# smups/inflatox

Hardware: AMD Instinct MI355X
Metric: grid-points/sec on complete_analysis sweep; achieved HBM GB/s vs peak (higher is better)
Workload: dtype f64

## Files before the change

### inflatox_amd/_native.py

```python

from __future__ import annotations

import ctypes as C
import os
import subprocess

import numpy as np

_PKG = os.path.dirname(os.path.abspath(__file__))
_REPO = os.path.dirname(_PKG)
LIB_PATH = os.path.join(_PKG, "libinflx_hip.so")

OK, ERR_IO, ERR_SYMBOL, ERR_VERSION, ERR_SHAPE, ERR_DEVICE, ERR_ARG, ERR_BASIS, ERR_GSL = range(9)
SF_EDOM, SF_EDECLINED = 1, 2
SF_QUIET, SF_FAIL = 0, 1

OP_COMPLETE, OP_CONSISTENCY, OP_RAPIDTURN, OP_EPSILON_V, OP_RAW = range(5)
OP_HESSE = 6
OP_QDIF = 5
OP_GROUP = {OP_COMPLETE: "core", OP_CONSISTENCY: "consistency", OP_RAPIDTURN: "rapidturn", OP_EPSILON_V: "epsilon_v", OP_RAW: "raw", OP_QDIF: "qdif", OP_HESSE: "hesse"}
OP_WIDTH = {OP_COMPLETE: 6, OP_CONSISTENCY: 1, OP_RAPIDTURN: 1, OP_EPSILON_V: 1, OP_RAW: 5, OP_HESSE: 4}
LAYOUT_AOS, LAYOUT_SOA = 0, 1
SWEEP_DEFAULT, SWEEP_FORCE_TILE = 0, 1
TIME_BACK_TO_BACK, TIME_DOMINANT_ONLY, TIME_IN_PIPELINE, TIME_SINGLE_CALL = range(4)
# ... 40 lines not shown
        C.c_int,
        [C.c_void_p, C.c_int, _DP, _SIZE, _SIZE, C.c_void_p, _SIZE, _DP, _SIZE, _SIZE, _SIZE, _SIZE, C.c_int, C.c_void_p, C.c_int, C.c_int, C.c_uint, C.POINTER(C.c_float)],
    ),
    "inflx_sweep_plan_ex": (C.c_int, [C.c_void_p, C.c_int, _SIZE, _SIZE, _SIZE, C.c_int, C.c_uint, C.POINTER(C.c_uint32)]),
    "inflx_host_threads": (C.c_int, [C.c_uint, C.POINTER(C.c_uint)]),
    "inflx_sweep_device_stats": (
        C.c_int,
        [C.c_void_p, _DP, _SIZE, _SIZE, C.c_void_p, _SIZE, _DP, _SIZE, _SIZE, _SIZE, _SIZE, C.c_void_p, C.c_void_p],
    ),
    "inflx_synchronize": (C.c_int, [C.c_void_p]),
    "inflx_sf_status": (C.c_int, [C.c_void_p, C.POINTER(C.c_uint), C.c_int]),
    "inflx_sf_policy": (C.c_int, [C.c_void_p, C.c_int]),
    "inflx_uses_gsl": (C.c_int, [C.c_void_p]),
    "inflx_sweep_plan": (C.c_int, [C.c_void_p, C.c_int, _SIZE, _SIZE, _SIZE, C.c_int, C.POINTER(C.c_uint32)]),
    "inflx_basis_on_points": (C.c_int, [C.c_void_p, _DP, _SIZE, _DP, _SIZE, _DP]),
    "inflx_ops_on_values": (C.c_int, [C.c_void_p, _DP, _SIZE, _DP, C.c_int]),
    "inflx_validate_basis_at_random": (C.c_int, [C.c_void_p, C.c_uint64]),
    "inflx_validate_basis_on_domain": (C.c_int, [C.c_void_p, C.POINTER(C.c_uint32), _SIZE, _DP, _SIZE, _DP, C.c_double]),
    "inflx_shard_plan": (C.c_int, [_SIZE, _SIZE, C.c_int, C.c_int, C.POINTER(_SIZE)]),
    "inflx_open_multi": (C.c_int, [C.c_char_p, C.POINTER(C.c_int), C.c_int, C.POINTER(C.c_void_p)]),
    "inflx_close_multi": (None, [C.c_void_p]),
    "inflx_multi_device_count": (C.c_int, [C.c_void_p]),
    "inflx_multi_handle": (C.c_void_p, [C.c_void_p, C.c_int]),
    "inflx_sweep_host_multi": (C.c_int, [C.c_void_p, C.c_int, _DP, _SIZE, _SIZE, _DP, _DP, _SIZE, _SIZE, C.c_int, C.c_int, _SIZE]),
    "inflx_complete_analysis_multi": (C.c_int, [C.c_void_p, _DP, _SIZE, _DP, _DP, _SIZE, _SIZE, C.c_int, _SIZE]),
    "inflx_sweep_stats_multi": (C.c_int, [C.c_void_p, _DP, _SIZE, _SIZE, _DP, _SIZE, _SIZE, _SIZE, C.c_void_p]),
    "inflx_sweep_device_multi": (C.c_int, [C.c_void_p, C.c_int, _DP, _SIZE, _SIZE, C.POINTER(C.c_void_p), C.POINTER(_SIZE), _DP, _SIZE, _SIZE, C.c_int, C.POINTER(C.c_void_p)]),
    "inflx_sweep_allgather_multi": (C.c_int, [C.c_void_p, C.c_int, _DP, _SIZE, _SIZE, C.POINTER(C.c_void_p), _SIZE, _DP, _SIZE, _SIZE]),
    "inflx_sweep_allgather_multi_ex": (C.c_int, [C.c_void_p, C.c_int, _DP, _SIZE, _SIZE, C.POINTER(C.c_void_p), _SIZE, _DP, _SIZE, _SIZE, C.c_int]),
    "inflx_solve_eom": (
        C.c_int,
        [C.c_void_p, _DP, _SIZE, _SIZE, _DP, _SIZE, _SIZE, _SIZE, C.c_int, C.c_double, C.c_double, C.c_uint, _DP, _DP, _DP, C.POINTER(C.c_int8), C.POINTER(C.c_int64)],
    ),
    "inflx_solve_eom_to_efolds": (
        C.c_int,
        [C.c_void_p, _DP, _SIZE, _SIZE, _DP, _SIZE, _DP, _SIZE, C.c_int, C.c_double, C.c_double, C.c_uint, _DP, _DP, _DP, _DP, C.POINTER(C.c_int8)],
    ),
    "inflx_solve_eom_sampled": (
        C.c_int,
        [C.c_void_p, _DP, _SIZE, _SIZE, _DP, _SIZE, _DP, _SIZE, _SIZE, C.c_int, C.c_double, C.c_double, C.c_uint, _DP, _DP, C.POINTER(C.c_int8), C.POINTER(C.c_uint32)],
    ),
}


class Summary(C.Structure):

    _fields_ = [("min", C.c_double * 6), ("max", C.c_double * 6), ("count", C.c_uint64 * 6)]

_lib = None


def build_library(force: bool = False) -> str:
    src = os.path.join(_PKG, "csrc", "inflx_hip.cpp")
    deps = [src, os.path.join(_PKG, "csrc", "inflx_kernel_abi.h"), os.path.join(_PKG, "csrc", "inflx_background_abi.h"), os.path.join(_REPO, "include", "inflx_hip.h")]
    stale = force or not os.path.exists(LIB_PATH) or any(os.path.getmtime(d) > os.path.getmtime(LIB_PATH) for d in deps)
    if stale:
        from .compiler import hipcc_path

        cmd = [
            hipcc_path(),
            "-O2",
            "-fPIC",
            "-shared",
            "-std=c++17",
            "-Wall",
            "-Wextra",
            f"-I{os.path.join(_REPO, 'include')}",
            f"-I{os.path.join(_PKG, 'csrc')}",
            src,
            "-o",
            LIB_PATH + ".tmp",
        ]
        subprocess.run(cmd, check=True)
        os.replace(LIB_PATH + ".tmp", LIB_PATH)
    return LIB_PATH


def _preload_hip_runtime():
    import importlib.util

    try:
        spec = importlib.util.find_spec("torch")
    except (ImportError, ValueError):
        spec = None
    if spec is not None and spec.origin:
        cand = os.path.join(os.path.dirname(spec.origin), "lib", "libamdhip64.so")
        if os.path.exists(cand):
            C.CDLL(cand, mode=C.RTLD_GLOBAL)


def load_library():
    global _lib
    if _lib is None:
        if not os.path.exists(LIB_PATH):
            raise ImportError(
                f"{LIB_PATH} is missing: build it with `python -c 'import __graft_entry__ as g; g.build()'` "
                "(the sweep has no CPU fallback)"
            )
        _preload_hip_runtime()
        lib = C.CDLL(LIB_PATH)
        for name, (res, args) in SIGNATURES.items():
            fn = getattr(lib, name)
            fn.restype = res
            fn.argtypes = args
        _lib = lib
    return _lib


class InflatoxShapeError(Exception):
    """Counterpart of LibInflxRsErr::Shape, which PyO3 raises as a plain Exception (err.rs:71)."""


class InflatoxBasisError(Exception):
    """Counterpart of LibInflxRsErr::BasisNorm / BasisOth (err.rs:36-37), plain Exceptions in PyO3 too."""


class InflatoxSpecialFunctionError(ArithmeticError):
    """A special function of the model was called outside its domain somewhere in the call (``INFLX_ERR_GSL``).  The reference's
    GSL error handler prints the reason and panics at that point (src/err.rs:86-103): the call does not return there either.  Here
    the result was complete when the error was raised -- NaN at the offending points -- and ``sf_errors="nan"`` returns it."""


def _raise(rc: int):
    msg = load_library().inflx_last_error().decode("utf-8", "replace")
    if rc == ERR_GSL:
        raise InflatoxSpecialFunctionError(msg)
    if rc == ERR_IO:
        raise IOError(msg)
# ... 469 lines not shown
```

### inflatox_amd/csrc/inflx_hip.cpp

```cpp
#include "inflx_hip.h"

#include <dlfcn.h>
#include <hip/hip_runtime.h>

#include <algorithm>
#include <atomic>
#include <cerrno>
#include <chrono>
#include <cmath>
#include <cstdarg>
#include <cstdio>
#include <cstdlib>
#include <condition_variable>
#include <cstring>
#include <mutex>
#include <future>
#include <random>
#include <string>
#include <thread>
#include <vector>

#include <sched.h>
#include <sys/mman.h>
#if defined(__x86_64__)
#include <emmintrin.h>
#endif
#include <unistd.h>

#include "inflx_background_abi.h"
#include "inflx_kernel_abi.h"

namespace {

thread_local std::string g_last_error;

int fail(int code, const char* fmt, ...) {
  char buf[1024];
  va_list ap;
  va_start(ap, fmt);
  vsnprintf(buf, sizeof buf, fmt, ap);
  va_end(ap);
  g_last_error = buf;
  return code;
}

#define HIP_TRY(expr)                                                                              \
  do {                                                                                             \
    hipError_t e_ = (expr);                                                                        \
    if (e_ != hipSuccess) return fail(INFLX_ERR_DEVICE, "%s failed: %s", #expr, hipGetErrorString(e_)); \
  } while (0)

constexpr uint16_t kAbiMajor = 5, kAbiMinor = 0;
const char* const kOpNames[INFLX_OP_COUNT] = {"complete", "consistency", "rapidturn", "epsilon_v", "raw", "qdif", "hesse"};
constexpr int kOpWidth[INFLX_OP_COUNT] = {6, 1, 1, 1, 5, 1, 4};
constexpr size_t kOpBytes[INFLX_OP_COUNT] = {48, 8, 8, 8, 40, 1, 32};

size_t chunk_bytes_limit() {
  static const size_t v = [] {
    const char* e = getenv("INFLX_CHUNK_MB");
    const long mb = e ? atol(e) : 0;
    return (size_t)(mb > 0 ? mb : 32) << 20;
  }();
  return v;
}
size_t whole_result_limit() {
  static const size_t v = [] {
    const char* e = getenv("INFLX_WHOLE_RESULT_MB");
    const long mb = e ? atol(e) : -1;
    return (size_t)(mb >= 0 ? mb : 65536) << 20;
  }();
  return v;
}
unsigned quota_from(const std::string& quota_file, const std::string& period_file) {
  FILE* fh = fopen(quota_file.c_str(), "r");
  if (!fh) return 0;
  char a[64] = {0}, b[64] = {0};
  const int got = fscanf(fh, "%63s %63s", a, b);
  fclose(fh);
  if (got < 1 || strcmp(a, "max") == 0) return 0;
  double quota = atof(a), period = got >= 2 ? atof(b) : 0.0;
  if (!period_file.empty()) {
    FILE* ph = fopen(period_file.c_str(), "r");
    if (!ph) return 0;
// ... 151 lines not shown
      }
    }
    if (!spawned) work(a, b);
  }
  for (auto& th : pool) th.join();
}

struct TableRing {
  double* buf[2] = {nullptr, nullptr};
  size_t cap[2] = {0, 0};
  hipEvent_t ready[2] = {nullptr, nullptr};
  hipEvent_t free[2] = {nullptr, nullptr};
  bool used[2] = {false, false};
  unsigned turn = 0;

  bool create() {
    for (int b = 0; b < 2; ++b)
      if (hipEventCreateWithFlags(&ready[b], hipEventDisableTiming | hipEventDisableSystemFence) != hipSuccess ||
          hipEventCreateWithFlags(&free[b], hipEventDisableTiming | hipEventDisableSystemFence) != hipSuccess)
        return false;
    return true;
  }
  void destroy() {
    for (int b = 0; b < 2; ++b) {
      if (ready[b]) (void)hipEventDestroy(ready[b]);
      if (free[b]) (void)hipEventDestroy(free[b]);
      if (buf[b]) (void)hipFree(buf[b]);
    }
  }
  bool idle() const {
    for (int b = 0; b < 2; ++b)
      if (used[b] && hipEventQuery(free[b]) != hipSuccess) return false;
    return true;
  }
  int grow(int b, size_t doubles) {
    if (buf[b]) HIP_TRY(hipFree(buf[b]));
    buf[b] = nullptr;
    cap[b] = 0;
    HIP_TRY(hipMalloc(reinterpret_cast<void**>(&buf[b]), doubles * sizeof(double)));
    cap[b] = doubles;
    return INFLX_OK;
  }
};
}

#define INFLX_SERIALISE(m) \
  std::unique_lock<std::recursive_mutex> inflx_call_lock_; \
  if (m) inflx_call_lock_ = std::unique_lock<std::recursive_mutex>((m)->mu)

struct inflx_model {
  std::recursive_mutex mu;
  int device = 0;
  hipModule_t module = nullptr;
  hipStream_t stream = nullptr;
  hipStream_t copy_stream = nullptr;
  hipFunction_t tile[INFLX_OP_COUNT] = {};
  hipFunction_t rows[INFLX_OP_COUNT] = {};
  hipFunction_t traj[INFLX_OP_COUNT] = {};
  hipFunction_t basis_points = nullptr;
  hipFunction_t ops_on_values = nullptr;
  hipFunction_t rowvals[INFLX_OP_COUNT] = {};
  hipFunction_t rowstream6 = nullptr;
  hipFunction_t rowstream_planes = nullptr;
  hipFunction_t colvals[INFLX_OP_COUNT] = {};
  hipFunction_t colstream = nullptr;
  hipFunction_t colvals_stats = nullptr;
  hipFunction_t stage_tables = nullptr;
  TableRing stage_ring;
  hipFunction_t tile_stats = nullptr, tile_stats_nostore = nullptr, rowvals_stats = nullptr;
  double* d_stats = nullptr;
  TableRing row_ring;
  hipStream_t side = nullptr;
  std::vector<std::pair<hipEvent_t, hipEvent_t>>* probe = nullptr;
  size_t probe_used = 0;
  bool probe_overflow = false;
  InflxKernelInfo info = {};
  uint32_t groups = 0;
  std::vector<hipModule_t> attached;
  std::string tag;
  std::vector<hipDeviceptr_t> sf_words;
  int sf_policy = INFLX_SF_QUIET;
  hipEvent_t sf_done = nullptr;
  bool sf_pending = false;
  char use_gsl = 0;
  uint16_t version[3] = {};
  uint32_t dim = 0, n_par = 0;
  std::string name, path;
  struct ParamSlot {
    double* host = nullptr;
    double* dev = nullptr;
    size_t cap = 0, count = 0;
    hipStream_t stream = nullptr;
    hipEvent_t last_use = nullptr;
    hipStream_t last_reader = nullptr;
    bool in_flight = false;
  };
  static constexpr int kParamSlots = 4;
  ParamSlot pslot[kParamSlots];
  int pcur = 0;
  void* d_chunk[2] = {nullptr, nullptr};
  size_t d_chunk_cap[2] = {0, 0};
  void* d_whole = nullptr;
  size_t d_whole_cap = 0;
  hipEvent_t chunk_done[2] = {nullptr, nullptr};
  hipEvent_t copy_done[2] = {nullptr, nullptr};
  hipEvent_t t0 = nullptr, t1 = nullptr;
// ... 71 lines not shown

void note_sf_word(inflx_model* m, hipModule_t module) {
  if (!m->use_gsl) return;
  hipDeviceptr_t dptr = nullptr;
  size_t size = 0;
  if (hipModuleGetGlobal(&dptr, &size, module, "INFLX_SF_STATUS") == hipSuccess && size == sizeof(unsigned))
    m->sf_words.push_back(dptr);
  else
    (void)hipGetLastError();
}

int sf_collect(inflx_model* m, bool clear, unsigned* bits) {
  *bits = 0;
  if (m->sf_words.empty()) return INFLX_OK;
  HIP_TRY(hipSetDevice(m->device));
  HIP_TRY(hipStreamSynchronize(m->side));
  HIP_TRY(hipStreamSynchronize(m->stream));
  if (m->sf_pending) {
    HIP_TRY(hipEventSynchronize(m->sf_done));
    m->sf_pending = false;
  }
  for (hipDeviceptr_t w : m->sf_words) {
    unsigned v = 0;
    HIP_TRY(hipMemcpy(&v, w, sizeof v, hipMemcpyDeviceToHost));
    *bits |= v;
    if (v && clear) {
      const unsigned zero = 0;
      HIP_TRY(hipMemcpy(w, &zero, sizeof zero, hipMemcpyHostToDevice));
    }
  }
  return INFLX_OK;
}

int sf_error(const inflx_model* m, unsigned bits) {
  const bool dom = (bits & INFLX_SF_EDOM) != 0;
  return fail(INFLX_ERR_GSL, "a GSL exception ocurred (ERRCODE %s): model \"%s\" called a special function %s at one or more points of this call. "
              "Those points hold NaN and the result is complete otherwise; the reference's GSL error handler panics here instead of returning. "
              "inflx_sf_policy(handle, INFLX_SF_QUIET) / GeneralisedAL(..., sf_errors=\"nan\") returns the result with its NaNs.",
              dom ? "0X1" : "0X11", m->name.c_str(),
              dom ? "outside its domain (input domain error)" : "where this implementation could not deliver 1e-13 and declined (loss of accuracy)");
}

int sf_verdict(inflx_model* m) {
  if (m->sf_words.empty() || m->sf_policy != INFLX_SF_FAIL) return INFLX_OK;
  unsigned bits = 0;
  const int rc = sf_collect(m, true, &bits);
  if (rc) return rc;
  return bits ? sf_error(m, bits) : INFLX_OK;
}

const char* const kGroupNames[9] = {"core", "stats", "values", "consistency", "rapidturn", "epsilon_v", "raw", "qdif", "hesse"};
uint32_t group_of_op(int op) { return INFLX_GROUP_OF_OP(op); }

int resolve_group_kernels(inflx_model* m, hipModule_t module, uint32_t mask, const char* path) {
  auto get = [&](hipFunction_t* slot, const std::string& name) -> int {
    if (hipModuleGetFunction(slot, module, name.c_str()) != hipSuccess) {
      *slot = nullptr;
      return fail(INFLX_ERR_SYMBOL, "artefact %s lacks kernel %s", path, name.c_str());
    }
    return INFLX_OK;
  };
  int rc;
  for (int op = 0; op < INFLX_OP_COUNT; ++op) {
    if (!(mask & group_of_op(op))) continue;
    const std::string nm = kOpNames[op];
    if ((rc = get(&m->tile[op], "inflx_sweep_tile_" + nm)) || (rc = get(&m->rows[op], "inflx_sweep_rows_" + nm)) || (rc = get(&m->traj[op], "inflx_sweep_traj_" + nm)) ||
        (rc = get(&m->rowvals[op], "inflx_sweep_rowvals_" + nm)) || (rc = get(&m->colvals[op], "inflx_sweep_colvals_" + nm)))
      return rc;
  }
  if (mask & INFLX_GROUP_CORE) {
    if ((rc = get(&m->rowstream6, "inflx_sweep_rowstream6")) || (rc = get(&m->rowstream_planes, "inflx_sweep_rowstream_planes")) || (rc = get(&m->colstream, "inflx_sweep_colstream")) ||
        (rc = get(&m->stage_tables, "inflx_stage_tables")) || (rc = get(&m->basis_points, "inflx_basis_points")))
      return rc;
  }
  if (mask & INFLX_GROUP_STATS) {
    if ((rc = get(&m->tile_stats, "inflx_sweep_tile_complete_stats")) || (rc = get(&m->tile_stats_nostore, "inflx_sweep_tile_complete_stats_nostore")) ||
        (rc = get(&m->rowvals_stats, "inflx_sweep_rowvals_complete_stats")) || (rc = get(&m->colvals_stats, "inflx_sweep_colvals_complete_stats")))
      return rc;
  }
  if (mask & INFLX_GROUP_VALUES) {
    if ((rc = get(&m->ops_on_values, "inflx_ops_on_values"))) return rc;
  }
  return INFLX_OK;
}

template <typename T>
int read_global_of(hipModule_t module, const char* path, const char* sym, T* dst, size_t bytes, bool exact) {
  hipDeviceptr_t dptr = nullptr;
  size_t size = 0;
  if (hipModuleGetGlobal(&dptr, &size, module, sym) != hipSuccess) return fail(INFLX_ERR_SYMBOL, "artefact %s lacks symbol %s", path, sym);
  if (exact ? size != bytes : size > bytes) return fail(INFLX_ERR_SYMBOL, "symbol %s in %s has %zu bytes, expected %s%zu", sym, path, size, exact ? "" : "<= ", bytes);
  HIP_TRY(hipMemcpy(dst, dptr, size, hipMemcpyDeviceToHost));
  return INFLX_OK;
}

int attach_object(inflx_model* m, const char* path) {
  hipModule_t module = nullptr;
  hipError_t e = hipModuleLoad(&module, path);
  if (e != hipSuccess) return fail(INFLX_ERR_IO, "could not load %s as a gfx950 code object: %s", path, hipGetErrorString(e));
  auto bail = [&](int code) {
    const std::string first = g_last_error;
    (void)hipModuleUnload(module);
    g_last_error = first;
    return code;
  };
  uint16_t version[3] = {};
  InflxKernelInfo info = {};
  uint32_t groups = 0;
  char tag[128] = {0};
  int rc;
  if ((rc = read_global_of(module, path, "VERSION", version, sizeof version, true)) || (rc = read_global_of(module, path, "INFLX_KERNEL_INFO", &info, sizeof info, true)) ||
      (rc = read_global_of(module, path, "INFLX_GROUPS", &groups, sizeof groups, true)) || (rc = read_global_of(module, path, "MODEL_TAG", tag, sizeof tag - 1, false)))
    return bail(rc);
  if (version[0] != m->version[0] || version[1] != m->version[1] || memcmp(&info, &m->info, sizeof info) != 0 || m->tag != tag)
    return bail(fail(INFLX_ERR_VERSION, "%s does not belong to artefact %s: built from another model, with other options or for another kernel ABI (tag \"%s\", expected \"%s\")",
                     path, m->path.c_str(), tag, m->tag.c_str()));
  const uint32_t fresh = groups & ~m->groups;
  if ((rc = resolve_group_kernels(m, module, fresh, path))) return bail(rc);
  m->attached.push_back(module);
  m->groups |= fresh;
  note_sf_word(m, module);
  return INFLX_OK;
}

int need_groups(inflx_model* m, uint32_t mask) {
// ... 61 lines not shown
    pl.cpr = (units_row + info.row_chunk_units - 1) / info.row_chunk_units;
    pl.replicas = 32;
    while (pl.replicas > 1 && pl.replicas > pl.cpr) pl.replicas /= 2;
    const size_t line_bytes = row_count * pl.replicas * 64;
    pl.batch = std::max<size_t>(1, std::min<size_t>(P, (size_t(64) << 20) / std::max<size_t>(line_bytes, 1)));
    pl.batch = std::min<size_t>(pl.batch, 65535 / (aos6 ? 1 : K));
    pl.one_stream = alone && P <= pl.batch;
  } else if (col_only && (planes ? N1 : K * N1) % 2 == 0) {
    pl.path = INFLX_PATH_COL_STREAM;
    pl.batch = std::max<size_t>(1, std::min<size_t>(P, (size_t(64) << 20) / std::max<size_t>(K * N1 * 8, 1)));
    pl.batch = std::min<size_t>(pl.batch, 65535 / (planes ? K : 1));
    pl.one_stream = alone && P <= pl.batch;
  } else if (row_only) {
    pl.path = INFLX_PATH_ROWS;
  } else {
    pl.path = INFLX_PATH_TILE;
    const size_t nu = std::max<size_t>(info.n_uniform, 1), nc = std::max<size_t>(info.n_col, 1);
    const size_t nr = (std::max<size_t>(info.n_row, 1) + 1) & ~size_t(1);
    pl.rows_per_launch = size_t(65535) * info.tile_rows;
    const size_t per_p = nu + std::min(pl.rows_per_launch, row_count) * nr + nc * N1;
    pl.batch = std::max<size_t>(1, std::min<size_t>(P, (size_t(1) << 27) / std::max<size_t>(per_p, 1)));
    pl.one_stream = alone && P <= pl.batch && row_count <= pl.rows_per_launch;
  }
  return pl;
}

bool handle_idle(inflx_model* m) {
  const bool idle = m->row_ring.idle() && m->stage_ring.idle();
  (void)hipGetLastError();
  return idle;
}

hipError_t probe_begin(inflx_model* m, hipStream_t s) {
  if (!m->probe) return hipSuccess;
  if (m->probe_used >= m->probe->size()) {
    m->probe_overflow = true;
    return hipSuccess;
  }
  return hipEventRecord((*m->probe)[m->probe_used].first, s);
}
hipError_t probe_end(inflx_model* m, hipStream_t s) {
  if (!m->probe || m->probe_used >= m->probe->size()) return hipSuccess;
  return hipEventRecord((*m->probe)[m->probe_used++].second, s);
}


struct BroadcastPath {
  hipFunction_t eval;
  unsigned eval_gx, eval_block;
  hipFunction_t store;
  size_t cpr;
  size_t z_per_p;
  size_t table_doubles;
};

int launch_broadcast(inflx_model* m, const SweepPlan& plan, const BroadcastPath& path, int op, InflxSweepArgs a, const double* d_params, size_t P,
                     double* d_out, hipStream_t s, bool stores_only) {
  void* params[] = {&a};
  TableRing& ring = m->row_ring;
  const hipStream_t ev = plan.upload_stream(m, s);
  const size_t batch = plan.batch, row_count = a.row_count;
  if (path.cpr > 0x7fffffffULL) return fail(INFLX_ERR_SHAPE, "grid rows too long for one launch");
  if (stores_only && batch < P)
    return fail(INFLX_ERR_ARG, "dominant_only timing needs the parameter rows to fit one table batch (%zu rows here, got %zu)", batch, P);
  const bool store = d_out != nullptr;
  for (size_t p0 = 0; p0 < P; p0 += batch) {
    const size_t pb = std::min(batch, P - p0);
    const int b = (int)((ring.turn + (stores_only ? 1 : 0)) & 1);
    if (store && pb * path.table_doubles > ring.cap[b]) {
      HIP_TRY(hipDeviceSynchronize());
      const int rc = ring.grow(b, pb * path.table_doubles);
      if (rc) return rc;
    }
    a.params = d_params + p0 * m->n_par;
    a.out = store ? d_out + p0 * row_count * a.N1 * kOpWidth[op] : nullptr;
    a.P = (uint32_t)pb;
    a.row_table = store ? ring.buf[b] : nullptr;
    if (!stores_only) {
      if (ring.used[b]) HIP_TRY(hipStreamWaitEvent(ev, ring.free[b], 0));
      HIP_TRY(hipModuleLaunchKernel(path.eval, path.eval_gx, (unsigned)pb, 1, path.eval_block, 1, 1, 0, ev, params, nullptr));
      if (ev != s) HIP_TRY(hipEventRecord(ring.ready[b], ev));
      ring.turn++;
    }
    if (store) {
      if (ev != s) HIP_TRY(hipStreamWaitEvent(s, ring.ready[b], 0));
      for (size_t r0 = 0; r0 < row_count; r0 += 65535) {
        a.stream_row0 = (uint32_t)r0;
        const size_t nr = std::min<size_t>(65535, row_count - r0);
        HIP_TRY(probe_begin(m, s));
        HIP_TRY(hipModuleLaunchKernel(path.store, (unsigned)path.cpr, (unsigned)nr, (unsigned)(pb * path.z_per_p), m->info.tile_cols, 1, 1, 0, s, params, nullptr));
        HIP_TRY(probe_end(m, s));
      }
      HIP_TRY(hipEventRecord(ring.free[b], s));
      ring.used[b] = true;
    }
  }
  return INFLX_OK;
}

int launch_rows_fallback(inflx_model* m, int op, InflxSweepArgs a, size_t P, size_t N1, size_t row_count, hipStream_t s) {
  void* params[] = {&a};
  const size_t rpb = m->info.rows_per_block;
  const size_t groups = (row_count + rpb - 1) / rpb;
  size_t chunks = 1;
  const size_t want = 4096;
  if (groups * P < want) {
    const size_t units = N1 / 64;
    chunks = std::min<size_t>(std::max<size_t>(units, 1), (want + groups * P - 1) / (groups * P));
  }
  if (groups * chunks > 0x7fffffffULL) return fail(INFLX_ERR_SHAPE, "grid too large for one launch");
  a.col_chunks = (uint32_t)chunks;
  HIP_TRY(hipModuleLaunchKernel(m->rows[op], (unsigned)(groups * chunks), (unsigned)P, 1, m->info.tile_cols, 1, 1, 0, s, params,
                                nullptr));
  return INFLX_OK;
}

constexpr size_t kLaunchWorkgroups = 1024;

size_t tile_height(size_t full, size_t segments) {
  return std::min(full, std::max<size_t>({size_t(1), std::min(full / 2, segments / kLaunchWorkgroups), segments / (4 * kLaunchWorkgroups)}));
}

int launch_tiles(inflx_model* m, const SweepPlan& plan, int op, InflxSweepArgs a, const double* d_params, size_t P, double* d_out, size_t N1,
                 size_t row_count, hipStream_t s, double* d_stats) {
  void* params[] = {&a};
  TableRing& ring = m->stage_ring;
  const size_t gx = (N1 + m->info.tile_cols - 1) / m->info.tile_cols;
  if (gx > 0x7fffffffULL) return fail(INFLX_ERR_SHAPE, "grid rows too long for one launch (%zu column tiles)", gx);
  if (row_count > 0xffffffffULL) return fail(INFLX_ERR_SHAPE, "at most 2^32 grid rows per call (got %zu)", row_count);
  hipFunction_t f = d_stats ? (d_out ? m->tile_stats : m->tile_stats_nostore) : m->tile[op];
  const size_t nu = std::max<size_t>(m->info.n_uniform, 1), nc = std::max<size_t>(m->info.n_col, 1);
  const size_t nr = (std::max<size_t>(m->info.n_row, 1) + 1) & ~size_t(1);
  const size_t rows_per_launch = plan.rows_per_launch, pbatch = plan.batch;
  const hipStream_t tables = plan.upload_stream(m, s);
  for (size_t p0 = 0; p0 < P; p0 += pbatch) {
    const size_t pb = std::min(pbatch, P - p0);
    a.params = d_params + p0 * m->n_par;
    a.out = d_out ? reinterpret_cast<double*>(reinterpret_cast<char*>(d_out) + p0 * row_count * N1 * kOpBytes[op]) : nullptr;
    a.P = (uint32_t)pb;
    for (size_t r0 = 0; r0 < row_count; r0 += rows_per_launch) {
      const size_t slab = std::min(rows_per_launch, row_count - r0);
      const size_t need = pb * (nu + slab * nr + nc * N1);
      const int b = (int)(ring.turn & 1);
// ... 10 lines not shown
      HIP_TRY(hipModuleLaunchKernel(m->stage_tables, (unsigned)tx, (unsigned)pb, 1, m->info.tile_cols, 1, 1, 0, tables, params, nullptr));
      ring.turn++;
      if (tables != s) {
        HIP_TRY(hipEventRecord(ring.ready[b], tables));
        HIP_TRY(hipStreamWaitEvent(s, ring.ready[b], 0));
      }
      const size_t th = tile_height(m->info.tile_rows, gx * slab * pb);
      a.tile_rows = (uint32_t)th;
      const size_t gy = (slab + th - 1) / th;
      HIP_TRY(probe_begin(m, s));
      HIP_TRY(hipModuleLaunchKernel(f, (unsigned)gx, (unsigned)gy, (unsigned)pb, m->info.tile_cols, 1, 1, 0, s, params, nullptr));
      HIP_TRY(probe_end(m, s));
      HIP_TRY(hipEventRecord(ring.free[b], s));
      ring.used[b] = true;
    }
  }
  return INFLX_OK;
}

int launch_grid(inflx_model* m, const SweepPlan& plan, int op, const double* d_params, size_t P, double* d_out, const double* ss, size_t N0,
                size_t N1, size_t row_begin, size_t row_count, int layout, hipStream_t s, bool stores_only = false, double accuracy = 0.0,
                double* d_stats = nullptr) {
  if (row_count == 0 || N1 == 0) return INFLX_OK;
  if (P > 65535) {
    for (size_t p0 = 0; p0 < P; p0 += 65535) {
      const size_t pb = std::min<size_t>(65535, P - p0);
      double* sub = d_out ? reinterpret_cast<double*>(reinterpret_cast<char*>(d_out) + p0 * row_count * N1 * kOpBytes[op]) : nullptr;
      const int rc = launch_grid(m, plan, op, d_params + p0 * m->n_par, pb, sub, ss, N0, N1, row_begin, row_count, layout, s, stores_only, accuracy, d_stats);
      if (rc) return rc;
    }
    return INFLX_OK;
  }
  InflxSweepArgs a;
  memset(&a, 0, sizeof a);
  a.out = d_out;
  a.params = d_params;
  a.x0a = ss[0];
  a.dx0 = (ss[1] - ss[0]) / (double)N0;
  a.x1a = ss[2];
  a.dx1 = (ss[3] - ss[2]) / (double)N1;
  a.N1 = N1;
  a.row_begin = row_begin;
  a.row_count = row_count;
  a.P = (uint32_t)P;
  a.layout = (uint32_t)layout;
  a.col_chunks = 1;
  a.accuracy = accuracy;
  a.stats = d_stats;
  const size_t K = kOpWidth[op];
  switch (plan.path) {
    case INFLX_PATH_ROW_STREAM: {
      const bool aos6 = K == 6 && layout == INFLX_AOS;
      a.table_replicas = (uint32_t)plan.replicas;
      a.stream_planes = (uint32_t)K;
      const BroadcastPath path = {d_stats ? m->rowvals_stats : m->rowvals[op], (unsigned)((row_count + 63) / 64), 64,
                                  aos6 ? m->rowstream6 : m->rowstream_planes, plan.cpr, aos6 ? 1 : K, row_count * plan.replicas * 8};
      return launch_broadcast(m, plan, path, op, a, d_params, P, d_out, s, stores_only);
    }
    case INFLX_PATH_COL_STREAM: {
      const bool planes = layout == INFLX_SOA || K == 1;
      a.stream_units = (planes ? N1 : K * N1) / 2;
      const size_t tc = m->info.tile_cols;
      const BroadcastPath path = {d_stats ? m->colvals_stats : m->colvals[op], (unsigned)((N1 + tc - 1) / tc), (unsigned)tc,
                                  m->colstream, (a.stream_units + tc - 1) / tc, planes ? K : 1, K * N1};
      return launch_broadcast(m, plan, path, op, a, d_params, P, d_out, s, stores_only);
    }
    case INFLX_PATH_ROWS:
      return launch_rows_fallback(m, op, a, P, N1, row_count, s);
    default:
      return launch_tiles(m, plan, op, a, d_params, P, d_out, N1, row_count, s, d_stats);
  }
}

int ensure_chunk(inflx_model* m, int which, size_t bytes) {
  if (bytes <= m->d_chunk_cap[which]) return INFLX_OK;
  if (m->d_chunk[which]) HIP_TRY(hipFree(m->d_chunk[which]));
  m->d_chunk[which] = nullptr;
  m->d_chunk_cap[which] = 0;
  HIP_TRY(hipMalloc(&m->d_chunk[which], bytes));
  m->d_chunk_cap[which] = bytes;
  return INFLX_OK;
}

void say(const char* fmt, ...) {
  va_list ap;
  va_start(ap, fmt);
  fputs("[Inflatox Info] ", stderr);
  vfprintf(stderr, fmt, ap);
  fputc('\n', stderr);
  fflush(stderr);
  va_end(ap);
}

void warn(const char* fmt, ...) {
  va_list ap;
  va_start(ap, fmt);
  fputs("[Inflatox Warning] ", stderr);
  vfprintf(stderr, fmt, ap);
  fputc('\n', stderr);
  fflush(stderr);
  va_end(ap);
}

std::string num_text(double v, int digits = -1) {
  if (std::isnan(v)) return "NaN";
  if (std::isinf(v)) return v > 0 ? "inf" : "-inf";
  char buf[64];
  if (digits >= 0) snprintf(buf, sizeof buf, "%.*f", digits, v); else snprintf(buf, sizeof buf, "%.17g", v);
  return buf;
}

std::string list_text(const double* v, size_t n) {
  std::string s = "[";
  for (size_t k = 0; k < n; ++k) s += (k ? ", " : "") + num_text(v[k], 3);
  return s + "]";
}

// ... 69 lines not shown
  if (device < 0 || device >= ndev) return fail(INFLX_ERR_ARG, "device %d out of range (have %d)", device, ndev);
  HIP_TRY(hipSetDevice(device));

  inflx_model* m = new inflx_model();
  m->device = device;
  m->path = artefact_path;
  auto bail = [&](int code) {
    inflx_close(m);
    return code;
  };
  hipError_t e = hipModuleLoad(&m->module, artefact_path);
  if (e != hipSuccess) {
    m->module = nullptr;
    fail(INFLX_ERR_IO, "could not load %s as a gfx950 code object: %s", artefact_path, hipGetErrorString(e));
    return bail(INFLX_ERR_IO);
  }
  int rc;
  if ((rc = read_global(m, "VERSION", m->version, sizeof m->version, true))) return bail(rc);
  if (m->version[0] != kAbiMajor || m->version[1] != kAbiMinor) {
    fail(INFLX_ERR_VERSION, "artefact %s was built for inflatox ABI v%u.%u.%u, this library implements v%u.%u", artefact_path,
         m->version[0], m->version[1], m->version[2], kAbiMajor, kAbiMinor);
    return bail(INFLX_ERR_VERSION);
  }
  if ((rc = read_global(m, "DIM", &m->dim, sizeof m->dim, true))) return bail(rc);
  if ((rc = read_global(m, "N_PARAMETERS", &m->n_par, sizeof m->n_par, true))) return bail(rc);
  char name[512] = {0};
  if ((rc = read_global(m, "MODEL_NAME", name, sizeof name - 1, false))) return bail(rc);
  m->name = name;
  if ((rc = read_global(m, "INFLX_KERNEL_INFO", &m->info, sizeof m->info, true))) return bail(rc);
  if (m->info.kernel_abi != INFLX_KERNEL_ABI) {
    fail(INFLX_ERR_VERSION, "artefact %s uses kernel ABI %u, this library expects %u", artefact_path, m->info.kernel_abi,
         INFLX_KERNEL_ABI);
    return bail(INFLX_ERR_VERSION);
  }
  if ((rc = read_global(m, "USE_GSL", &m->use_gsl, sizeof m->use_gsl, true))) return bail(rc);
  note_sf_word(m, m->module);
  m->sf_policy = m->use_gsl ? INFLX_SF_FAIL : INFLX_SF_QUIET;
  char tag[128] = {0};
  if ((rc = read_global(m, "INFLX_GROUPS", &m->groups, sizeof m->groups, true))) return bail(rc);
  if ((rc = read_global(m, "MODEL_TAG", tag, sizeof tag - 1, false))) return bail(rc);
  m->tag = tag;
  m->groups &= INFLX_GROUP_ALL;
  if (!(m->groups & INFLX_GROUP_CORE)) {
    fail(INFLX_ERR_SYMBOL, "artefact %s is not a model's core object (it carries kernel groups 0x%x only): open the core object and attach this one (inflx_attach)", artefact_path, m->groups);
    m->groups = 0;
    return bail(INFLX_ERR_SYMBOL);
  }
  {
    const uint32_t present = m->groups;
    m->groups = 0;
    if ((rc = resolve_group_kernels(m, m->module, present, artefact_path))) return bail(rc);
    m->groups = present;
  }
  if (hipStreamCreateWithFlags(&m->stream, hipStreamNonBlocking) != hipSuccess ||
      hipStreamCreateWithFlags(&m->side, hipStreamNonBlocking) != hipSuccess ||
      hipStreamCreateWithFlags(&m->copy_stream, hipStreamNonBlocking) != hipSuccess) {
    fail(INFLX_ERR_DEVICE, "could not create HIP streams");
    return bail(INFLX_ERR_DEVICE);
  }
  for (int k = 0; k < 2; ++k) {
    if (hipEventCreateWithFlags(&m->chunk_done[k], hipEventDisableTiming) != hipSuccess ||
        hipEventCreateWithFlags(&m->copy_done[k], hipEventDisableTiming) != hipSuccess) {
      fail(INFLX_ERR_DEVICE, "could not create HIP events");
      return bail(INFLX_ERR_DEVICE);
    }
  }
  for (TableRing* ring : {&m->row_ring, &m->stage_ring}) {
    if (!ring->create()) {
      fail(INFLX_ERR_DEVICE, "could not create HIP events");
      return bail(INFLX_ERR_DEVICE);
    }
  }
  if (hipEventCreate(&m->t0) != hipSuccess || hipEventCreate(&m->t1) != hipSuccess) {
    fail(INFLX_ERR_DEVICE, "could not create HIP timing events");
    return bail(INFLX_ERR_DEVICE);
  }
  *out = m;
  return INFLX_OK;
}

void inflx_close(inflx_model* m) {
  if (!m) return;
  { std::lock_guard<std::recursive_mutex> last_call_has_returned(m->mu); }
  (void)hipSetDevice(m->device);
  if (m->stream) (void)hipStreamSynchronize(m->stream);
  if (m->side) (void)hipStreamSynchronize(m->side);
  if (m->copy_stream) (void)hipStreamSynchronize(m->copy_stream);
  for (int k = 0; k < 2; ++k) {
    if (m->d_chunk[k]) (void)hipFree(m->d_chunk[k]);
    if (m->chunk_done[k]) (void)hipEventDestroy(m->chunk_done[k]);
    if (m->copy_done[k]) (void)hipEventDestroy(m->copy_done[k]);
  }
  for (TableRing* ring : {&m->row_ring, &m->stage_ring}) ring->destroy();
  if (m->t0) (void)hipEventDestroy(m->t0);
  if (m->t1) (void)hipEventDestroy(m->t1);
  if (m->sf_done) (void)hipEventDestroy(m->sf_done);
  for (auto& slot : m->pslot) {
    if (slot.dev) (void)hipFree(slot.dev);
    if (slot.host) (void)hipHostFree(slot.host);
    if (slot.last_use) (void)hipEventDestroy(slot.last_use);
  }
  if (m->d_stats) (void)hipFree(m->d_stats);
  if (m->d_whole) (void)hipFree(m->d_whole);
  if (m->stream) (void)hipStreamDestroy(m->stream);
  if (m->side) (void)hipStreamDestroy(m->side);
  if (m->copy_stream) (void)hipStreamDestroy(m->copy_stream);
  for (hipModule_t extra : m->attached) (void)hipModuleUnload(extra);
  if (m->bg_module) (void)hipModuleUnload(m->bg_module);
  if (m->module) (void)hipModuleUnload(m->module);
  delete m;
}

int inflx_attach(inflx_model* m, const char* path) {
  if (!m || !path) return fail(INFLX_ERR_ARG, "model handle / path is NULL");
  INFLX_SERIALISE(m);
  FILE* fh = fopen(path, "rb");
  if (!fh) return fail(INFLX_ERR_IO, "could not open code object %s: %s", path, strerror(errno));
  fclose(fh);
  HIP_TRY(hipSetDevice(m->device));
  return attach_object(m, path);
}

uint32_t inflx_groups(const inflx_model* m) { return m ? m->groups : 0; }

uint32_t inflx_n_fields(const inflx_model* m) { return m ? m->dim : 0; }
uint32_t inflx_n_parameters(const inflx_model* m) { return m ? m->n_par : 0; }
const char* inflx_model_name(const inflx_model* m) { return m ? m->name.c_str() : ""; }
int inflx_device_of(const inflx_model* m) { return m ? m->device : -1; }

int inflx_host_threads(unsigned devices_at_work, unsigned out[3]) {
  if (!out) return fail(INFLX_ERR_ARG, "output array is NULL");
  const unsigned saved = tl_sharers;
  tl_sharers = std::max(1u, devices_at_work);
  out[0] = host_cpu_budget();
  out[1] = prefault_threads();
  out[2] = host_fill_threads();
  tl_sharers = saved;
  return INFLX_OK;
}

int inflx_stage_info(const inflx_model* m, uint32_t* nu, uint32_t* nr, uint32_t* nc, uint32_t* out_mask) {
  if (!m) return fail(INFLX_ERR_ARG, "model handle is NULL");
  if (nu) *nu = m->info.n_uniform;
  if (nr) *nr = m->info.n_row;
  if (nc) *nc = m->info.n_col;
  if (out_mask) *out_mask = m->info.out_mask;
  return INFLX_OK;
}

int inflx_sweep_plan(const inflx_model* m, int op, size_t P, size_t N1, size_t row_count, int layout, uint32_t plan[4]) {
  return inflx_sweep_plan_ex(m, op, P, N1, row_count, layout, INFLX_SWEEP_DEFAULT, plan);
}

int inflx_sweep_plan_ex(const inflx_model* m, int op, size_t P, size_t N1, size_t row_count, int layout, unsigned flags, uint32_t plan[4]) {
  if (!m || !plan) return fail(INFLX_ERR_ARG, "model handle / plan array is NULL");
  if (op < 0 || op >= INFLX_OP_COUNT) return fail(INFLX_ERR_ARG, "unknown sweep operation %d", op);
  if (flags & ~(unsigned)INFLX_SWEEP_FORCE_TILE) return fail(INFLX_ERR_ARG, "unknown sweep flags 0x%x", flags);
  const SweepPlan pl = plan_sweep(m->info, op, layout, P, N1, row_count, flags, false);
  plan[0] = (uint32_t)pl.path;
  plan[1] = plan[2] = plan[3] = 0;
  if (pl.path == INFLX_PATH_ROWS) return INFLX_OK;
// ... 1679 lines not shown
```

Before: 150.9 billion.

## Move store-stream kernels into a separate gfx950 code object with nontemporal stores

Builds the row/column broadcast store kernels as their own gfx950 code object, compiled at -O3 with kernarg preloading. They write through inline-asm global_store_dwordx4 with sc1 nt cache hints and use scalar table loads plus a packed argument struct. The host loads this module at open time and passes precomputed pitch, replica shift/mask and plane-division multipliers, replacing the artefact's own stream kernels. The aim is to cut store overhead and cache pollution on the dominant HBM write stream. In exchange it hardcodes gfx950 and adds a second module that must match the artefact's thread count.

```diff
diff --git a/inflatox_amd/_native.py b/inflatox_amd/_native.py
--- a/inflatox_amd/_native.py
+++ b/inflatox_amd/_native.py
@@ -116,7 +116,7 @@
 
 def build_library(force: bool = False) -> str:
     src = os.path.join(_PKG, "csrc", "inflx_hip.cpp")
-    deps = [src, os.path.join(_PKG, "csrc", "inflx_kernel_abi.h"), os.path.join(_PKG, "csrc", "inflx_background_abi.h"), os.path.join(_REPO, "include", "inflx_hip.h")]
+    deps = [src, os.path.join(_PKG, "csrc", "inflx_kernel_abi.h"), os.path.join(_PKG, "csrc", "inflx_stream_abi.h"), os.path.join(_PKG, "csrc", "inflx_background_abi.h"), os.path.join(_REPO, "include", "inflx_hip.h")]
     stale = force or not os.path.exists(LIB_PATH) or any(os.path.getmtime(d) > os.path.getmtime(LIB_PATH) for d in deps)
     if stale:
         from .compiler import hipcc_path
@@ -137,7 +137,39 @@
         ]
         subprocess.run(cmd, check=True)
         os.replace(LIB_PATH + ".tmp", LIB_PATH)
+    _build_stream_kernels(force)
     return LIB_PATH
+
+
+STREAM_KERNELS_PATH = os.path.join(os.path.dirname(LIB_PATH), "inflx_stream_kernels.hsaco")
+
+
+def _build_stream_kernels(force: bool = False) -> str:
+    src = os.path.join(_PKG, "csrc", "inflx_stream_kernels.hip")
+    deps = [src, os.path.join(_PKG, "csrc", "inflx_stream_abi.h")]
+    out = STREAM_KERNELS_PATH
+    if force or not os.path.exists(out) or any(os.path.getmtime(d) > os.path.getmtime(out) for d in deps):
+        from .compiler import hipcc_path
+
+        cmd = [
+            hipcc_path(),
+            "--offload-arch=gfx950",
+            "--genco",
+            "--no-gpu-bundle-output",
+            "-O3",
+            "-std=c++17",
+            "-Wall",
+            "-Werror",
+            "-mllvm",
+            "-amdgpu-kernarg-preload-count=16",
+            f"-I{os.path.join(_PKG, 'csrc')}",
+            src,
+            "-o",
+            out + f".{os.getpid()}.tmp",
+        ]
+        subprocess.run(cmd, check=True)
+        os.replace(out + f".{os.getpid()}.tmp", out)
+    return out
 
 
 def _preload_hip_runtime():
diff --git a/inflatox_amd/csrc/inflx_hip.cpp b/inflatox_amd/csrc/inflx_hip.cpp
--- a/inflatox_amd/csrc/inflx_hip.cpp
+++ b/inflatox_amd/csrc/inflx_hip.cpp
@@ -29,6 +29,7 @@
 
 #include "inflx_background_abi.h"
 #include "inflx_kernel_abi.h"
+#include "inflx_stream_abi.h"
 
 namespace {
 
@@ -286,6 +287,7 @@
   std::recursive_mutex mu;
   int device = 0;
   hipModule_t module = nullptr;
+  hipModule_t stream_module = nullptr;
   hipStream_t stream = nullptr;
   hipStream_t copy_stream = nullptr;
   hipFunction_t tile[INFLX_OP_COUNT] = {};
@@ -463,6 +465,35 @@
 const char* const kGroupNames[9] = {"core", "stats", "values", "consistency", "rapidturn", "epsilon_v", "raw", "qdif", "hesse"};
 uint32_t group_of_op(int op) { return INFLX_GROUP_OF_OP(op); }
 
+int load_stream_kernels(inflx_model* m) {
+  std::string path = "inflx_stream_kernels.hsaco";
+  Dl_info self;
+  if (dladdr(reinterpret_cast<const void*>(&inflx_last_error), &self) && self.dli_fname) {
+    const std::string lib = self.dli_fname;
+    const size_t slash = lib.rfind('/');
+    if (slash != std::string::npos) path = lib.substr(0, slash + 1) + path;
+  }
+  hipError_t e = hipModuleLoad(&m->stream_module, path.c_str());
+  if (e != hipSuccess) {
+    m->stream_module = nullptr;
+    return fail(INFLX_ERR_IO, "could not load the store-stream kernels %s as a gfx950 code object: %s", path.c_str(), hipGetErrorString(e));
+  }
+  InflxStreamInfo info = {};
+  hipDeviceptr_t dptr = nullptr;
+  size_t size = 0;
+  if (hipModuleGetGlobal(&dptr, &size, m->stream_module, "INFLX_STREAM_INFO") != hipSuccess || size != sizeof info ||
+      hipMemcpy(&info, dptr, sizeof info, hipMemcpyDeviceToHost) != hipSuccess)
+    return fail(INFLX_ERR_SYMBOL, "%s has no INFLX_STREAM_INFO", path.c_str());
+  if (info.stream_abi != INFLX_STREAM_ABI || info.threads != m->info.tile_cols || info.threads != m->info.row_chunk_units)
+    return fail(INFLX_ERR_VERSION, "%s uses stream ABI %u with %u threads, this library expects %u and the artefact %u", path.c_str(), info.stream_abi,
+                info.threads, INFLX_STREAM_ABI, m->info.tile_cols);
+  struct { hipFunction_t* f; const char* name; } const want[] = {
+      {&m->rowstream6, "inflx_sweep_rowstream6"}, {&m->rowstream_planes, "inflx_sweep_rowstream_planes"}, {&m->colstream, "inflx_sweep_colstream"}};
+  for (const auto& w : want)
+    if (hipModuleGetFunction(w.f, m->stream_module, w.name) != hipSuccess) return fail(INFLX_ERR_SYMBOL, "%s lacks kernel %s", path.c_str(), w.name);
+  return INFLX_OK;
+}
+
 int resolve_group_kernels(inflx_model* m, hipModule_t module, uint32_t mask, const char* path) {
   auto get = [&](hipFunction_t* slot, const std::string& name) -> int {
     if (hipModuleGetFunction(slot, module, name.c_str()) != hipSuccess) {
@@ -480,8 +511,7 @@
       return rc;
   }
   if (mask & INFLX_GROUP_CORE) {
-    if ((rc = get(&m->rowstream6, "inflx_sweep_rowstream6")) || (rc = get(&m->rowstream_planes, "inflx_sweep_rowstream_planes")) || (rc = get(&m->colstream, "inflx_sweep_colstream")) ||
-        (rc = get(&m->stage_tables, "inflx_stage_tables")) || (rc = get(&m->basis_points, "inflx_basis_points")))
+    if ((rc = get(&m->stage_tables, "inflx_stage_tables")) || (rc = get(&m->basis_points, "inflx_basis_points")))
       return rc;
   }
   if (mask & INFLX_GROUP_STATS) {
@@ -649,6 +679,8 @@
   size_t cpr;
   size_t z_per_p;
   size_t table_doubles;
+  size_t units_row;
+  size_t replicas;
 };
 
 int launch_broadcast(inflx_model* m, const SweepPlan& plan, const BroadcastPath& path, int op, InflxSweepArgs a, const double* d_params, size_t P,
@@ -657,7 +689,18 @@
   TableRing& ring = m->row_ring;
   const hipStream_t ev = plan.upload_stream(m, s);
   const size_t batch = plan.batch, row_count = a.row_count;
-  if (path.cpr > 0x7fffffffULL) return fail(INFLX_ERR_SHAPE, "grid rows too long for one launch");
+  if (path.cpr > 0x7fffffffULL || path.units_row > 0xffffff00ULL) return fail(INFLX_ERR_SHAPE, "grid rows too long for one launch");
+  if (row_count > 0xffffffffULL) return fail(INFLX_ERR_SHAPE, "at most 2^32 grid rows per call (got %zu)", row_count);
+  InflxStreamArgs st;
+  memset(&st, 0, sizeof st);
+  st.pitch = (uint64_t)path.units_row * 16;
+  st.units_row = (uint32_t)path.units_row;
+  st.rows_per_p = (uint32_t)row_count;
+  for (size_t r = path.replicas; r > 1; r /= 2) st.rep_shift++;
+  st.rep_mask = path.replicas ? (uint32_t)path.replicas - 1 : 0;
+  st.planes = (uint32_t)path.z_per_p;
+  st.plane_mul = (uint32_t)(((size_t(1) << 20) + path.z_per_p - 1) / path.z_per_p);
+  void* stream_params[] = {&st.out, &st.table, &st.pitch, &st.units_row, &st.rows_per_p, &st.rep_shift, &st.rep_mask, &st.planes, &st.plane_mul};
   if (stores_only && batch < P)
     return fail(INFLX_ERR_ARG, "dominant_only timing needs the parameter rows to fit one table batch (%zu rows here, got %zu)", batch, P);
   const bool store = d_out != nullptr;
@@ -682,10 +725,11 @@
     if (store) {
       if (ev != s) HIP_TRY(hipStreamWaitEvent(s, ring.ready[b], 0));
       for (size_t r0 = 0; r0 < row_count; r0 += 65535) {
-        a.stream_row0 = (uint32_t)r0;
+        st.out = a.out + r0 * path.units_row * 2;
+        st.table = a.row_table + r0 * path.replicas * 8;
         const size_t nr = std::min<size_t>(65535, row_count - r0);
         HIP_TRY(probe_begin(m, s));
-        HIP_TRY(hipModuleLaunchKernel(path.store, (unsigned)path.cpr, (unsigned)nr, (unsigned)(pb * path.z_per_p), m->info.tile_cols, 1, 1, 0, s, params, nullptr));
+        HIP_TRY(hipModuleLaunchKernel(path.store, (unsigned)path.cpr, (unsigned)nr, (unsigned)(pb * path.z_per_p), m->info.tile_cols, 1, 1, 0, s, stream_params, nullptr));
         HIP_TRY(probe_end(m, s));
       }
       HIP_TRY(hipEventRecord(ring.free[b], s));
@@ -802,17 +846,17 @@
     case INFLX_PATH_ROW_STREAM: {
       const bool aos6 = K == 6 && layout == INFLX_AOS;
       a.table_replicas = (uint32_t)plan.replicas;
-      a.stream_planes = (uint32_t)K;
       const BroadcastPath path = {d_stats ? m->rowvals_stats : m->rowvals[op], (unsigned)((row_count + 63) / 64), 64,
-                                  aos6 ? m->rowstream6 : m->rowstream_planes, plan.cpr, aos6 ? 1 : K, row_count * plan.replicas * 8};
+                                  aos6 ? m->rowstream6 : m->rowstream_planes, plan.cpr, aos6 ? 1 : K, row_count * plan.replicas * 8,
+                                  aos6 ? 3 * N1 : N1 / 2, plan.replicas};
       return launch_broadcast(m, plan, path, op, a, d_params, P, d_out, s, stores_only);
     }
     case INFLX_PATH_COL_STREAM: {
       const bool planes = layout == INFLX_SOA || K == 1;
-      a.stream_units = (planes ? N1 : K * N1) / 2;
+      const size_t units = (planes ? N1 : K * N1) / 2;
       const size_t tc = m->info.tile_cols;
       const BroadcastPath path = {d_stats ? m->colvals_stats : m->colvals[op], (unsigned)((N1 + tc - 1) / tc), (unsigned)tc,
-                                  m->colstream, (a.stream_units + tc - 1) / tc, planes ? K : 1, K * N1};
+                                  m->colstream, (units + tc - 1) / tc, planes ? K : 1, K * N1, units, 0};
       return launch_broadcast(m, plan, path, op, a, d_params, P, d_out, s, stores_only);
     }
     case INFLX_PATH_ROWS:
@@ -988,6 +1032,7 @@
     if ((rc = resolve_group_kernels(m, m->module, present, artefact_path))) return bail(rc);
     m->groups = present;
   }
+  if ((rc = load_stream_kernels(m))) return bail(rc);
   if (hipStreamCreateWithFlags(&m->stream, hipStreamNonBlocking) != hipSuccess ||
       hipStreamCreateWithFlags(&m->side, hipStreamNonBlocking) != hipSuccess ||
       hipStreamCreateWithFlags(&m->copy_stream, hipStreamNonBlocking) != hipSuccess) {
@@ -1043,6 +1088,7 @@
   if (m->copy_stream) (void)hipStreamDestroy(m->copy_stream);
   for (hipModule_t extra : m->attached) (void)hipModuleUnload(extra);
   if (m->bg_module) (void)hipModuleUnload(m->bg_module);
+  if (m->stream_module) (void)hipModuleUnload(m->stream_module);
   if (m->module) (void)hipModuleUnload(m->module);
   delete m;
 }
diff --git a/inflatox_amd/csrc/inflx_stream_abi.h b/inflatox_amd/csrc/inflx_stream_abi.h
--- /dev/null
+++ b/inflatox_amd/csrc/inflx_stream_abi.h
@@ -0,0 +1,22 @@
+#pragma once
+#include <stdint.h>
+
+#define INFLX_STREAM_ABI 1u
+#define INFLX_STREAM_THREADS 256u
+
+struct InflxStreamArgs {
+  double* out;
+  const double* table;
+  uint64_t pitch;
+  uint32_t units_row;
+  uint32_t rows_per_p;
+  uint32_t rep_shift;
+  uint32_t rep_mask;
+  uint32_t planes;
+  uint32_t plane_mul;
+};
+
+struct InflxStreamInfo {
+  uint32_t stream_abi;
+  uint32_t threads;
+};
diff --git a/inflatox_amd/csrc/inflx_stream_kernels.hip b/inflatox_amd/csrc/inflx_stream_kernels.hip
--- /dev/null
+++ b/inflatox_amd/csrc/inflx_stream_kernels.hip
@@ -0,0 +1,79 @@
+#include <hip/hip_runtime.h>
+#include <stdint.h>
+
+#include "inflx_stream_abi.h"
+
+constexpr unsigned kThreads = INFLX_STREAM_THREADS;
+typedef double inflx_d2 __attribute__((ext_vector_type(2)));
+
+extern "C" __device__ __attribute__((used, visibility("default"))) InflxStreamInfo INFLX_STREAM_INFO = {INFLX_STREAM_ABI, INFLX_STREAM_THREADS};
+
+#ifndef INFLX_STREAM_STORE
+#define INFLX_STREAM_STORE 1
+#endif
+__device__ __forceinline__ void stream_store_d2(char* base, unsigned off, inflx_d2 v) {
+#if INFLX_STREAM_STORE == 0
+  __builtin_nontemporal_store(v, reinterpret_cast<inflx_d2*>(base + off));
+#elif INFLX_STREAM_STORE == 1
+  asm volatile("global_store_dwordx4 %0, %1, %2 sc1 nt" : : "v"(off), "v"(v), "s"(base) : "memory");
+#elif INFLX_STREAM_STORE == 2
+  asm volatile("global_store_dwordx4 %0, %1, %2 sc0 sc1 nt" : : "v"(off), "v"(v), "s"(base) : "memory");
+#elif INFLX_STREAM_STORE == 3
+  asm volatile("global_store_dwordx4 %0, %1, %2 sc1" : : "v"(off), "v"(v), "s"(base) : "memory");
+#else
+  asm volatile("global_store_dwordx4 %0, %1, %2 sc0 sc1" : : "v"(off), "v"(v), "s"(base) : "memory");
+#endif
+}
+
+#define INFLX_STREAM_PARAMS                                                                                                      \
+  double *out, const double *table, uint64_t pitch, uint32_t units_row, uint32_t rows_per_p, uint32_t rep_shift, uint32_t rep_mask, \
+      uint32_t planes, uint32_t plane_mul
+
+__device__ __forceinline__ char* stream_piece(double* out, uint64_t out_row, uint64_t pitch, unsigned piece) {
+  uint64_t off = out_row * pitch + (uint64_t)piece * (kThreads * 16);
+  asm("" : "+s"(off));
+  return reinterpret_cast<char*>(out) + off;
+}
+
+__device__ __forceinline__ const double* stream_entry(const double* table, unsigned slab_row, unsigned piece, unsigned rep_shift, unsigned rep_mask) {
+  return table + ((((uint64_t)slab_row << rep_shift) + (piece & rep_mask)) << 3);
+}
+
+extern "C" __global__ __launch_bounds__(kThreads) void inflx_sweep_rowstream6(INFLX_STREAM_PARAMS) {
+  const unsigned k = blockIdx.x;
+  const unsigned slab_row = blockIdx.z * rows_per_p + blockIdx.y;
+  const double* __restrict__ t = stream_entry(table, slab_row, k, rep_shift, rep_mask);
+  const unsigned u = k * kThreads + threadIdx.x;
+  unsigned phase = (k % 3 + threadIdx.x) % 3;
+  asm("" : "+v"(phase));
+  char* const dst = stream_piece(out, slab_row, pitch, k);
+  double t0 = t[0], t1 = t[1], t2 = t[2], t3 = t[3], t4 = t[4], t5 = t[5];
+  asm volatile("" : "+s"(t0), "+s"(t1), "+s"(t2), "+s"(t3), "+s"(t4), "+s"(t5));
+  const inflx_d2 v = {phase == 0 ? t0 : (phase == 1 ? t2 : t4), phase == 0 ? t1 : (phase == 1 ? t3 : t5)};
+  if (u < units_row) stream_store_d2(dst, threadIdx.x * 16u, v);
+}
+static_assert(kThreads % 3 == 1, "the phase rule of inflx_sweep_rowstream6 needs kThreads == 1 (mod 3)");
+
+extern "C" __global__ __launch_bounds__(kThreads) void inflx_sweep_rowstream_planes(INFLX_STREAM_PARAMS) {
+  const unsigned piece = blockIdx.x;
+  const unsigned z = blockIdx.z;
+  const unsigned p = (unsigned)(((uint64_t)z * plane_mul) >> 20);
+  const unsigned k = z - p * planes;
+  const unsigned slab_row = p * rows_per_p + blockIdx.y;
+  const double* __restrict__ t = stream_entry(table, slab_row, piece, rep_shift, rep_mask);
+  double v = t[k];
+  const unsigned u = piece * kThreads + threadIdx.x;
+  char* const dst = stream_piece(out, (uint64_t)z * rows_per_p + blockIdx.y, pitch, piece);
+  asm volatile("" : "+s"(v));
+  if (u < units_row) stream_store_d2(dst, threadIdx.x * 16u, inflx_d2{v, v});
+}
+
+extern "C" __global__ __launch_bounds__(kThreads) void inflx_sweep_colstream(INFLX_STREAM_PARAMS) {
+  const unsigned piece = blockIdx.x;
+  const unsigned u = piece * kThreads + threadIdx.x;
+  const uint64_t z = blockIdx.z;
+  if (u < units_row) {
+    const inflx_d2 v = (reinterpret_cast<const inflx_d2*>(table) + z * units_row)[u];
+    stream_store_d2(stream_piece(out, z * rows_per_p + blockIdx.y, pitch, piece), threadIdx.x * 16u, v);
+  }
+}
```

After: 151.9 billion, median of 6. No clear change (+0.7%).
